# eriq-augustine/KB2E

Measured on AMD Instinct MI355X. Metric: training triples/sec (1/2/4/8 MI355X) + FB15k Hits@10(Filter), higher is better.
Workload: dtype f64

## Files before the change

### kb2e_amd/csrc/engine_transr_parallel.inc

```
namespace {

constexpr int32_t kRParLongMin = 128;

template <typename T, bool P, bool G>
const void* tile_fn(int nb) {
    switch (nb) {
        case 1: return (const void*)transr_tile_mfma_kernel<T, P, G, 1>;
        case 2: return (const void*)transr_tile_mfma_kernel<T, P, G, 2>;
        case 3: return (const void*)transr_tile_mfma_kernel<T, P, G, 3>;
        case 4: return (const void*)transr_tile_mfma_kernel<T, P, G, 4>;
        case 5: return (const void*)transr_tile_mfma_kernel<T, P, G, 5>;
        case 6: return (const void*)transr_tile_mfma_kernel<T, P, G, 6>;
        case 7: return (const void*)transr_tile_mfma_kernel<T, P, G, 7>;
        case 8: return (const void*)transr_tile_mfma_kernel<T, P, G, 8>;
    }
    throw std::runtime_error("TransR tile kernel: n > 128");
}

template <typename T>
const void* cons_tile_fn(int nb) {
    switch (nb) {
        case 1: return (const void*)transr_cons_tile_kernel<T, 1>;
        case 2: return (const void*)transr_cons_tile_kernel<T, 2>;
        case 3: return (const void*)transr_cons_tile_kernel<T, 3>;
// ... 214 lines not shown
        const std::pair<DevBuf*, DevBuf*> sets[] = {
            {&c->sb_x, &c->xreal}, {&c->sb_d, &c->aux}, {&c->sb_y, &c->rpar_y}, {&c->sb_wpart, &c->rpar_wpart},
            {&c->sb_rpart, &c->rpar_rpart}, {&c->sb_pflag, &c->rpar_pflag}, {&c->sb_cons_tile, &c->rpar_cons_tile},
            {&c->sb_cpairs, &c->rpar_cpairs}, {&c->sb_vio, &c->rpar_vio}, {&c->sb_cnrows, &c->rpar_cnrows}};
        for (const auto& pr : sets) {
            pr.first->free();
            if (c->sub > 1 && !c->rpar_merge_a && pr.second->p) {
                pr.first->alloc(pr.second->bytes);
                memset_sync(pr.first->p, 0, pr.first->bytes);
            }
        }
    }
    for (const void* k : {(const void*)rpar_scan_energy_kernel<double>, (const void*)rpar_scan_energy_kernel<float>,
                          (const void*)rpar_scan_energy_merged_kernel<double>,
                          (const void*)rpar_scan_energy_merged_kernel<float>})
        (void)hipFuncSetAttribute(k, hipFuncAttributeMaxDynamicSharedMemorySize, (int)rpar_scan_lds(c));
    (void)hipGetLastError();
}

void build_transr_tiles(kb2e_ctx* c, bool tiles, hipStream_t st, int set) {
    const int64_t nkeys = c->S * c->slots;
    rtile_count_kernel<<<1024, 256, 0, st>>>(c->keys_sorted.as<uint64_t>(), c->seg_start.as<int32_t>(),
                                                    c->nseg.as<int32_t>(), nkeys + 1, c->kl, c->cfg.num_entities,
                                                    c->rpar_St, c->rpar_ntiles.as<int32_t>(),
                                                    c->rpar_rel_begin.as<int32_t>());
    HIPCHK(hipGetLastError());
    if (!tiles) return;
    size_t tb = c->sort_tmp_bytes;
    HIPCHK(hipcub::DeviceScan::ExclusiveSum(c->sort_tmp.p, tb, c->rpar_ntiles.as<int32_t>(),
                                            c->rpar_tile_first.as<int32_t>(), (int)(nkeys + 1), st));
    rtile_scatter_kernel<<<1024, 256, 0, st>>>(c->rpar_ntiles.as<int32_t>(), c->rpar_tile_first.as<int32_t>(),
                                                      c->nseg.as<int32_t>(), c->rpar_tiles.as<RTile>());
    HIPCHK(hipGetLastError());
    if (c->rpar_brel.p) {
        rel_list_kernel<<<(int)c->nbi, 1024, 0, st>>>(c->rpar_rel_begin.as<int32_t>(), c->batch_seg.as<int32_t>(),
                                                     c->seg_row.as<int32_t>(), c->cfg.num_entities,
                                                     c->rel_order.as<int32_t>(), c->cfg.num_relations,
                                                     c->rpar_brel_cap, c->rpar_brel.as<int32_t>(),
                                                     c->rpar_bnrel.as<int32_t>());
        HIPCHK(hipGetLastError());
        HIPCHK(hipMemcpyAsync(c->pin_bnrel, c->rpar_bnrel.p, (size_t)c->nbi * 4, hipMemcpyDeviceToHost, st));
    }
    if (c->rpar_td_r.p) {
        RTileDescArgs d{};
        d.keys = c->keys_sorted.as<uint64_t>();
        d.seg_start = c->seg_start.as<int32_t>();
        d.seg_row = c->seg_row.as<int32_t>();
        d.tiles = c->rpar_tiles.as<RTile>();
        d.tile_first = c->rpar_tile_first.as<int32_t>();
        d.nseg = c->nseg.as<int32_t>();
        d.batch_seg = c->batch_seg.as<int32_t>();
        d.nb = (int32_t)c->nbi;
        d.sub = c->sub;
        d.Bs = (int32_t)c->Bs;
        d.St = c->rpar_St;
        d.ne = c->cfg.num_entities;
        d.B = (int32_t)c->B;
        d.kl = c->kl;
        d.si = c->si_[set].as<int32_t>();
        d.sj = c->sj_[set].as<int32_t>();
        d.side = c->side_[set].as<uint8_t>();
        d.heads = c->heads.as<int32_t>();
        d.tails = c->tails.as<int32_t>();
        d.batch_t0 = c->rpar_batch_t0.as<int32_t>();
        d.td_r = c->rpar_td_r.as<int32_t>();
        d.td_cnt = c->rpar_td_cnt.as<int32_t>();
        d.td_kk = c->rpar_td_kk.as<int32_t>();
        d.td_ent = c->rpar_td_ent.as<int32_t>();
        rtile_desc_kernel<<<2048, 256, 0, st>>>(d);
        HIPCHK(hipGetLastError());
    }
}

DevBuf& buf_set(int set, DevBuf& s0, DevBuf& s1) { return set ? s1 : s0; }

bool sub_overlap_on() {
    const char* e = getenv("KB2E_SUB_OVERLAP");
    return !(e && e[0] == '0');
}

int32_t pipe_opt_bits() {
    const char* e = getenv("KB2E_RPAR_PIPE_OPT");
    return e && e[0] ? (int32_t)(atoi(e) & kPipeOptAll) : kPipeOptAll;
}

constexpr int32_t kRecDeferChunks = 12;
int32_t rec_defer_chunks() {
    const char* e = getenv("KB2E_RPAR_REC_DEFER");
    return e && e[0] ? std::max(0, atoi(e)) : kRecDeferChunks;
}

template <typename T>
void fill_rpar(kb2e_ctx* c, int64_t b, int j, int set, RParArgs& a, RParBufs<T>& bf) {
    const int64_t ib = b * c->sub + j;
    const int64_t first = b * c->B + (int64_t)j * c->Bs;
    const int64_t cnt = std::min<int64_t>(c->Bs, c->B - (int64_t)j * c->Bs);
    a = RParArgs{};
    a.heads = c->heads.as<int32_t>();
    a.tails = c->tails.as<int32_t>();
    a.rels = c->rels.as<int32_t>();
    a.si = c->si() + first;
    a.sj = c->sj() + first;
    a.side = c->side() + first;
    a.B = (int32_t)cnt;
    a.n = c->n;
    a.ld = c->ld;
    a.ne = c->cfg.num_entities;
    a.nr = c->cfg.num_relations;
    a.St = c->rpar_St;
    a.tgroup = c->rpar_tgroup;
    a.batch = (int32_t)ib;
    a.lr = c->cfg.learning_rate;
    a.margin = c->cfg.margin;
    a.compat = c->cfg.transr_compat;
    a.l1 = c->cfg.distance == 0;
    a.keys = c->keys_sorted.as<uint64_t>();
    a.seg_start = c->seg_start.as<int32_t>();
    a.batch_seg = c->batch_seg.as<int32_t>();
    a.seg_row = c->seg_row.as<int32_t>();
    a.rel_begin = c->rpar_rel_begin.as<int32_t>();
    a.tile_first = c->rpar_tile_first.as<int32_t>();
    a.tiles = c->rpar_tiles.as<RTile>();
    a.kl = c->kl;
    a.act = c->act.as<uint8_t>() + first;
    a.loss = c->loss.as<double>() + first;
    a.proj = c->aux2.as<double>();
    a.tile_act = c->rpar_tile_act.as<int32_t>();
    a.batch_t0 = c->rpar_batch_t0.as<int32_t>();
    a.td_r = c->rpar_td_r.as<int32_t>();
    a.td_cnt = c->rpar_td_cnt.as<int32_t>();
    a.td_kk = c->rpar_td_kk.as<int32_t>();
    a.td_ent = c->rpar_td_ent.as<int32_t>();
    a.brel = c->rpar_brel.as<int32_t>() + ib * c->rpar_brel_cap;
    a.nrel = c->pin_bnrel[ib];
    if (a.nrel < 1 || a.nrel > c->rpar_brel_cap) throw std::logic_error("batch relation count out of range");
    bf = RParBufs<T>{};
    bf.ent = c->ent.as<T>();
    bf.rel = c->rel.as<T>();
    bf.W = c->w.as<T>();
    bf.x = buf_set(set, c->xreal, c->sb_x).as<T>();
    bf.d = buf_set(set, c->aux, c->sb_d).as<T>();
    bf.y = buf_set(set, c->rpar_y, c->sb_y).as<T>();
    bf.wpart = buf_set(set, c->rpar_wpart, c->sb_wpart).as<T>();
    bf.rpart = buf_set(set, c->rpar_rpart, c->sb_rpart).as<T>();
    bf.pair = c->rpar_pair.as<T>();
    bf.relpair = c->rpar_relpair.as<T>();
    bf.relpair_stamp = c->rpar_relpair_stamp.as<uint32_t>();
    bf.err = c->dataflow_err.as<uint32_t>() + 1;
    if (c->rpar_mfma) {
        bf.pflag = buf_set(set, c->rpar_pflag, c->sb_pflag).as<uint8_t>();
        bf.cons_tile = buf_set(set, c->rpar_cons_tile, c->sb_cons_tile).as<int32_t>();
        bf.cons_ppt = c->rpar_cons_wave ? kConsPpt : 1;
        bf.cpairs = buf_set(set, c->rpar_cpairs, c->sb_cpairs).as<int32_t>();
        bf.vio = buf_set(set, c->rpar_vio, c->sb_vio).as<int32_t>();
        bf.cnrows = buf_set(set, c->rpar_cnrows, c->sb_cnrows).as<int32_t>();
        bf.stats = getenv("KB2E_RPAR_STATS") != nullptr;
        bf.last_renorm = c->rpar_cons_seq ? 1 : 0;
        if (const char* dbg = getenv("KB2E_CONS_DBG")) bf.dbg = atoi(dbg);
        if (const char* cl = getenv("KB2E_RPAR_CHAIN_LIST")) bf.chain_list = std::max(64, atoi(cl));
        if (const char* ct = getenv("KB2E_RPAR_CHAIN_TILES")) bf.chain_tiles = std::max(1, atoi(ct));
        if (const char* rc = getenv("KB2E_RPAR_REC_CAP")) bf.rec_cap = std::max(4, atoi(rc));
        bf.pipe_opt = pipe_opt_bits();
        if (c->rpar_cons_seq) {
            bf.rec_stamp = bf.relpair_stamp + c->cfg.num_relations;
            bf.rec_defer = rec_defer_chunks();
        }
    }
    if (c->rpar_cons_wide || c->rpar_cons_gen || c->rpar_widep) {
        bf.pflag = buf_set(set, c->rpar_pflag, c->sb_pflag).as<uint8_t>();
        if (const char* dbg = getenv("KB2E_CONS_DBG")) bf.dbg = atoi(dbg);
        bf.stats = getenv("KB2E_RPAR_STATS") != nullptr;
        bf.last_renorm = 1;
    }
}

template <typename T>
void transr_phase_b(kb2e_ctx* c, RParArgs a, RParBufs<T> bf);

template <typename T>
void run_subbatch_transr_parallel(kb2e_ctx* c, int64_t b, int j) {
    const bool ov = c->sub > 1 && sub_overlap_on();
    const bool side = ov && j > 0;
    const int set = ov ? (j & 1) : 0;
    hipStream_t sa = side ? c->suba_stream : c->stream;
    RParArgs a;
    RParBufs<T> bf;
    fill_rpar<T>(c, b, j, set, a, bf);
    {
        unsigned long long* t0 = c->rpar_ptab.as<unsigned long long>();
        const size_t sz = (size_t)c->rpar_ptab_mask + 1;
        a.ptab = t0 + (c->batch_stamp % 3) * sz;
        a.ptab_next = t0 + ((c->batch_stamp + 1) % 3) * sz;
        a.ptab_mask = c->rpar_ptab_mask;
    }
    bf.stamp = ++c->batch_stamp;
    RParBufs<T> bfa = bf;
    if (c->sub > 1) {
        bfa.ent = c->snap_ent.as<T>();
        bfa.rel = c->snap_rel.as<T>();
        bfa.W = c->snap_w.as<T>();
    }
    if (side && j == 1) HIPCHK(hipStreamWaitEvent(sa, c->ev_adone[0], 0));
    if (side && j >= 2) HIPCHK(hipStreamWaitEvent(sa, c->ev_bdone[set], 0));
    auto a_done = [&] {
        if (!ov) return;
        HIPCHK(hipEventRecord(c->ev_adone[set], sa));
        if (side) HIPCHK(hipStreamWaitEvent(c->stream, c->ev_adone[set], 0));
    };
    auto b_done = [&] {
        if (ov) HIPCHK(hipEventRecord(c->ev_bdone[set], c->stream));
    };
    if (c->rpar_widep) {
        c->timed_on(sa, "score", [&] {
            wide_phase_a<T>(a, bfa, c->rpar_wg, c->rpar_max_tiles, c->rpar_scan.as<double>(),
                            c->rpar_scan_pre.as<double>(), c->transr_work.as<double>(),
                            c->transr_work_alt.as<double>(), sa);
        });
        if (c->cfg.transr_compat) std::swap(c->transr_work.p, c->transr_work_alt.p);
        a_done();
        c->timed("apply", [&] {
            wide_phase_b<T>(a, bf, c->rpar_wg, c->rpar_wsc.as<double>(), !c->rpar_no_constraint,
                            (int)std::min<int64_t>(c->cfg.num_relations, c->Bs), c->stream);
        });
        b_done();
        if (c->pending.size() > 4096) c->flush_timers();
        return;
    }
    const size_t lds = rpar_lds<T>(c);
    const int tgrid = c->rpar_max_tiles;
    const bool mf = c->rpar_mfma;
    const size_t lt = mf ? rmfma_lds<T>(c, false) : lds;
// ... 183 lines not shown
```

### kb2e_amd/csrc/kernels_transr_parallel.hpp

```cpp
#pragma once

#include <type_traits>

#include "kernels_common.hpp"

namespace kb2e {

struct RTile {
    int32_t seg, q;
};

struct RParArgs {
    const int32_t* heads;
    const int32_t* tails;
    const int32_t* rels;
    const int32_t* si;
    const int32_t* sj;
    const uint8_t* side;
    int32_t B, n, ld, ne, nr, St;
    int32_t batch;
    int32_t tgroup;
    double lr, margin;
    int32_t compat, l1;
    const uint64_t* keys;
// ... 62 lines not shown
__device__ __forceinline__ unsigned long long ptab_key(int r, int e) {
    return ((unsigned long long)r << kPtabEntBits) | (unsigned long long)e;
}
__device__ __forceinline__ uint32_t ptab_hash(int r, int e) {
    return ((uint32_t)e * 2654435761u) ^ ((uint32_t)r * 0x9E3779B1u + 0x7F4A7C15u);
}

__device__ __forceinline__ void ptab_insert(const RParArgs& a, int r, int e, int slot) {
    const unsigned long long key = ptab_key(r, e);
    const unsigned long long word = (key << kPtabSlotBits) | (unsigned long long)slot;
    uint32_t h = ptab_hash(r, e) & a.ptab_mask;
    while (true) {
        const unsigned long long old = atomicCAS(a.ptab + h, kPtabEmpty, word);
        if (old == kPtabEmpty) return;
        if ((old >> kPtabSlotBits) == key) {
            atomicMin(a.ptab + h, word);
            return;
        }
        h = (h + 1) & a.ptab_mask;
    }
}

__device__ __forceinline__ int ptab_first(const RParArgs& a, int r, int e) {
    const unsigned long long key = ptab_key(r, e);
    uint32_t h = ptab_hash(r, e) & a.ptab_mask;
    while (true) {
        const unsigned long long w = a.ptab[h];
        if (w == kPtabEmpty) return -1;
        if ((w >> kPtabSlotBits) == key) return (int)(w & ((1ull << kPtabSlotBits) - 1));
        h = (h + 1) & a.ptab_mask;
    }
}

__device__ __forceinline__ void ptab_clear_next(const RParArgs& a, int64_t tid, int64_t nthreads) {
    for (int64_t q = tid; q <= (int64_t)a.ptab_mask; q += nthreads) a.ptab_next[q] = kPtabEmpty;
}

__device__ __forceinline__ bool transr_pair_dup(const RParArgs& a, int slot, int r, int e) {
    return ptab_first(a, r, e) < slot;
}
__device__ __forceinline__ bool transr_relpair_dup(const RParArgs& a, int r) {
    return ptab_first(a, r, r) >= 0;
}

static __attribute__((unused)) __global__ __launch_bounds__(256) void transr_pair_first_kernel(RParArgs a) {
    const int slot = blockIdx.x * blockDim.x + threadIdx.x;
    ptab_clear_next(a, slot, (int64_t)gridDim.x * blockDim.x);
    if (slot >= 4 * a.B) return;
    const int kk = slot >> 2, u = (slot >> 1) & 1, role = slot & 1;
    if (!a.act[kk]) return;
    const int i0 = a.si[kk], jj = a.sj[kk];
    const int h = a.heads[i0], tt = a.tails[i0];
    const int hh = u ? (a.side[kk] ? h : jj) : h;
    const int th = u ? (a.side[kk] ? jj : tt) : tt;
    ptab_insert(a, a.rels[i0], role ? th : hh, slot);
}

template <typename T>
struct RParBufs {
    T* ent;
    T* rel;
    T* W;
    T* x;
    T* d;
    T* y;
    T* wpart;
    T* rpart;
    T* pair;
    T* relpair;
    uint32_t* relpair_stamp;
    uint32_t stamp;
    uint8_t* pflag;
    int32_t* cons_tile;
    int32_t cons_ppt;
    int32_t* cpairs;
    int32_t* cnrows;
    int32_t stats;
    int32_t last_renorm;
    int32_t dbg;
    int32_t chain_list;
    int32_t chain_tiles;
    int32_t rec_cap;
    int32_t pipe_opt;
    int32_t* vio;
    uint32_t* err;
    uint32_t* rec_stamp;
    int32_t rec_defer;
};

constexpr int32_t kPipeOptHandover = 2, kPipeOptDefer = 8, kPipeOptPublish = 16;
constexpr int32_t kPipeOptAll = kPipeOptHandover | kPipeOptDefer | kPipeOptPublish;

__host__ __device__ constexpr int rm_up16_host_dev(int v) { return (v + 15) & ~15; }
constexpr int kCPairs = 64;

struct RParMerge {
    int32_t sub;
    int32_t Bs;
    int32_t Blast;
    int32_t tcap;
    int32_t nch;
    int32_t brel_cap;
};

template <typename P>
__host__ __device__ __forceinline__ void rpar_advance(P*& p, int64_t k) {
    if (p) p += k;
}

template <typename T>
__host__ __device__ __forceinline__ void rpar_sub_view(RParArgs& a, RParBufs<T>& bf, const RParMerge& m, int j) {
    const int64_t s0 = (int64_t)j * m.Bs, t0 = (int64_t)j * m.tcap;
    a.B = j == m.sub - 1 ? m.Blast : m.Bs;
    a.batch += j;
    rpar_advance(a.si, s0);
    rpar_advance(a.sj, s0);
    rpar_advance(a.side, s0);
    rpar_advance(a.act, s0);
    rpar_advance(a.loss, s0);
    rpar_advance(a.proj, s0 * 4 * a.ld);
    rpar_advance(a.brel, (int64_t)j * m.brel_cap);
    rpar_advance(a.ptab, (int64_t)j * ((int64_t)a.ptab_mask + 1));
    rpar_advance(bf.x, s0 * 2 * a.ld);
    rpar_advance(bf.d, s0 * 2 * a.ld);
    rpar_advance(bf.y, s0 * 2 * a.ld);
    rpar_advance(bf.pflag, s0 * 4);
    rpar_advance(bf.wpart, t0 * bf.cons_ppt * a.n * a.ld);
    rpar_advance(bf.rpart, t0 * a.ld);
    rpar_advance(bf.cons_tile, t0 * bf.cons_ppt);
    rpar_advance(bf.cpairs, t0 * 2 * kCPairs);
    rpar_advance(bf.vio, t0 * kCPairs);
    rpar_advance(bf.cnrows, t0);
}

__device__ __forceinline__ void ptab_clear_group(const RParArgs& a, int sub, int64_t tid, int64_t nthreads) {
    const int64_t words = (int64_t)sub * ((int64_t)a.ptab_mask + 1);
    for (int64_t q = tid; q < words; q += nthreads) a.ptab_next[q] = kPtabEmpty;
}

template <typename T>
__host__ __device__ constexpr int rpar_lds_w(int n, int ld) {
    return n * ld;
}

__device__ __forceinline__ void tile_range(const RParArgs& a, int t, int& r, int& e0, int& cnt) {
    const RTile tl = a.tiles[t];
    const int p0 = a.seg_start[tl.seg], p1 = a.seg_start[tl.seg + 1];
    r = a.seg_row[tl.seg] - a.ne;
    const int ns = (p1 - p0) / 2;
    const int f = tl.q * a.St;
    e0 = p0 + 2 * f;
    cnt = min(a.St, ns - f);
}

template <typename T>
__device__ __forceinline__ void stage_matrix(T* Wl, const T* Wg, int n, int ld) {
    for (int idx = threadIdx.x; idx < n * ld; idx += blockDim.x) Wl[idx] = Wg[idx];
}

template <typename T>
__device__ __forceinline__ void project4(const T* Wl, int ld, int n, const T* v4 , T (&p)[4][2]) {
    const int l = lane_id();
    const int i = 2 * l;
#pragma unroll
    for (int q = 0; q < 4; ++q) p[q][0] = p[q][1] = T(0);
    if (i >= n) return;
    for (int j = 0; j < n; ++j) {
        const T w0 = Wl[j * ld + i], w1 = Wl[j * ld + i + 1];
#pragma unroll
        for (int q = 0; q < 4; ++q) {
            const T vj = v4[q * ld + j];
            p[q][0] += w0 * vj;
            p[q][1] += w1 * vj;
        }
// ... 369 lines not shown
        } else if (!transr_relpair_dup(a, r)) {
            ent = r;
        }
        ent_of[pq] = ent;
    }
    stage_matrix(Wl, bf.W + (int64_t)r * n * ld, n, ld);
    __syncthreads();
    T* v4 = vec + w * 4 * ld;
    const int i = 2 * l;
    for (int pq = w; pq < npairs; pq += 4) {
        const int ent = ent_of[pq];
        bool live = ent >= 0;
        for (int k = 0; live && k < pq; ++k) live = ent_of[k] != ent;
        T a0[2] = {T(0), T(0)}, G[2] = {T(0), T(0)}, da[2] = {T(0), T(0)};
        if (live) {
            lane_pair_load(bf.ent + (int64_t)ent * ld, n, a0);
            const T s0 = wave_sum(a0[0] * a0[0] + a0[1] * a0[1]);
            lane_pair_store(v4, n, a0);
            wave_lds_sync();
            T p[2] = {T(0), T(0)};
            if (i < n)
                for (int j = 0; j < n; ++j) {
                    const T aj = v4[j];
                    p[0] += Wl[j * ld + i] * aj;
                    p[1] += Wl[j * ld + i + 1] * aj;
                }
            if (i + 1 >= n) p[1] = T(0);
            if (i >= n) p[0] = T(0);
            wave_lds_sync();
            for (int m = 0; m < kRParMaxIter; ++m) {
                const T xx = wave_sum(p[0] * p[0] + p[1] * p[1]);
                if (!(xx > T(1))) break;
                G[0] += T(2) * p[0];
                G[1] += T(2) * p[1];
                lane_pair_store(v4, n, p);
                wave_lds_sync();
                T v[2];
                matvec_rows(Wl, ld, n, v4, v);
                lane_pair_store(v4 + ld, n, v);
                wave_lds_sync();
                T q[2] = {T(0), T(0)};
                if (i < n)
                    for (int j = 0; j < n; ++j) {
                        const T vj = v4[ld + j];
                        q[0] += Wl[j * ld + i] * vj;
                        q[1] += Wl[j * ld + i + 1] * vj;
                    }
                wave_lds_sync();
                const T c = T(2) * T(a.lr) * s0;
#pragma unroll
                for (int k = 0; k < 2; ++k) p[k] = i + k < n ? p[k] - T(2) * T(a.lr) * q[k] - c * p[k] : T(0);
            }
            lane_pair_store(v4, n, G);
            wave_lds_sync();
            matvec_rows(Wl, ld, n, v4, da);
            da[0] *= T(-a.lr);
            da[1] *= T(-a.lr);
            wave_lds_sync();
        }
        if (pq < 4 * cnt) {
            const int q = pq >> 2, u = (pq >> 1) & 1, role = pq & 1;
            const int kk = a.kl.kk_of(a.keys[e0 + 2 * q]);
            if (a.act[kk]) lane_pair_store(bf.pair + (((int64_t)kk * 2 + u) * 2 + role) * ld, n, da);
        } else {
            lane_pair_store(bf.relpair + (int64_t)r * ld, n, da);
            if (l == 0) bf.relpair_stamp[r] = bf.stamp;
        }
        const T dv[2] = {T(-a.lr) * a0[0], T(-a.lr) * a0[1]};
        lane_pair_store(Xl + pq * ld, n, G);
        lane_pair_store(Dl + pq * ld, n, dv);
    }
    __syncthreads();
    T* wp = bf.wpart + (int64_t)blockIdx.x * n * ld;
    for (int j = w; j < n; j += 4) {
        T acc[2];
        rank_sum_rows(Dl, Xl, npairs, ld, n, j, acc);
        lane_pair_store(wp + (int64_t)j * ld, n, acc);
    }
}

constexpr int kRParWaves = 16;

constexpr int kRecSteps = 4;
template <typename T>
__device__ __forceinline__ void rpar_record_convert(const RParArgs& a, const RParBufs<T>& bf, int r, T (&v)[2]) {
    typedef T T2 __attribute__((ext_vector_type(2)));
    const int n = a.n, l = lane_id();
    const T2* wrow = (const T2*)(bf.W + ((int64_t)r * n + (l < n ? l : 0)) * a.ld);
    const int nq = (n + 1) >> 1;
    T acc[4] = {T(0), T(0), T(0), T(0)};
    for (int q0 = 0; 2 * q0 < n; q0 += 2 * kRecSteps) {
        T2 x[2 * kRecSteps];
#pragma unroll
        for (int q = 0; q < 2 * kRecSteps; ++q) x[q] = wrow[q0 + q < nq ? q0 + q : nq - 1];
#pragma unroll
        for (int q = 0; q < 2 * kRecSteps; ++q) {
            const int i = 2 * (q0 + q);
            const T g0 = readlane_f(v[0], (q0 + q) & (kWave - 1)), g1 = readlane_f(v[1], (q0 + q) & (kWave - 1));
            acc[(2 * q) & 3] = fma(i < n ? x[q].x : T(0), g0, acc[(2 * q) & 3]);
            acc[(2 * q + 1) & 3] = fma(i + 1 < n ? x[q].y : T(0), g1, acc[(2 * q + 1) & 3]);
        }
    }
    const T da = -(T)a.lr * ((acc[0] + acc[1]) + (acc[2] + acc[3]));
    const T d0 = __shfl(da, (2 * l) & (kWave - 1)), d1 = __shfl(da, (2 * l + 1) & (kWave - 1));
    v[0] = 2 * l < n ? d0 : T(0);
    v[1] = 2 * l + 1 < n ? d1 : T(0);
}

__device__ __forceinline__ int rpar_entity_last(const RParArgs& a, int p0, int p1, int first, int stride) {
    const int l = lane_id();
    int last = -1;
    for (int base = p0 + first * kWave; base < p1; base += stride * kWave) {
        const int p = base + l;
        if (p < p1) {
            const uint64_t key = a.keys[p];
            const int kk = a.kl.kk_of(key);
            if (a.act[kk] && (key & (kRoleHead | kRoleTail))) last = max(last, kk * 2 + (int)((key >> 3) & 1));
        }
    }
#pragma unroll
    for (int s = 32; s >= 1; s >>= 1) last = max(last, __shfl_xor(last, s));
    return last;
}

template <typename T, bool GRAD>
__device__ __forceinline__ void rpar_entity_events(const RParArgs& a, const RParBufs<T>& bf, int row, int p0, int p1,
                                                   int first, int stride, int last, T (&acc)[2], T (&acc2)[2],
                                                   bool& dirty, bool& dirty2, bool& er_seen) {
    const int n = a.n, ld = a.ld, l = lane_id();
    const bool split = !GRAD && bf.last_renorm;
    const bool defer = !GRAD && bf.rec_stamp != nullptr;
    for (int base = p0 + first * kWave; base < p1; base += stride * kWave) {
        const int p = base + l;
        int src = -1;
        int src2 = -1;
        int rdef = -1;
        T c = T(0);
        bool nrm = false, er = false, post = false;
        if (p < p1) {
            const uint64_t key = a.keys[p];
            const int kk = a.kl.kk_of(key);
            if (a.act[kk]) {
                const int u = (int)((key >> 3) & 1);
                const uint32_t roles = (uint32_t)(key & 7);
                const bool hd = roles & kRoleHead, tl = roles & kRoleTail;
                er = roles & kRoleEntRel;
                if (GRAD) {
                    nrm = hd || tl;
                    if (hd != tl) {
                        src = kk * 2 + u;
                        c = (T)((hd ? -1.0 : 1.0) * (u ? 1.0 : -1.0) * a.lr);
                    }
                } else {
                    const int s0 = (kk * 2 + u) * 2;
                    const bool ph = hd && (!bf.pflag || bf.pflag[s0]);
                    const bool pt = tl && (!bf.pflag || bf.pflag[s0 + 1]);
                    nrm = ph || pt;
                    post = split && kk * 2 + u == last;
                    if (ph) src = s0;
                    if (pt) {
                        if (src < 0) src = s0 + 1;
                        else src2 = s0 + 1;
                    }
                    if (defer && src >= 0) {
                        const int r = a.rels[a.si[kk]];
                        if (bf.rec_stamp[r] == bf.stamp) rdef = r;
                    }
                }
            }
        }
        if (__ballot(nrm && !post)) dirty = true;
        if (__ballot(nrm && post)) dirty2 = true;
        if (__ballot(er)) er_seen = true;
        const T* tab = GRAD ? bf.y : bf.pair;
        for (int pass = 0; pass < (GRAD ? 1 : 2); ++pass) {
            const int mine = pass ? src2 : src;
            uint64_t m = __ballot(mine >= 0);
            const uint64_t pm = __ballot(post);
            while (m) {
                int ev[4];
                int k = 0;
                for (; k < 4 && m; ++k) {
                    ev[k] = __builtin_ctzll(m);
                    m &= m - 1;
                }
                T v[4][2];
#pragma unroll
                for (int q = 0; q < 4; ++q)
                    if (q < k) lane_pair_load(tab + (int64_t)readlane_i32(mine, ev[q]) * ld, n, v[q]);
                if (defer && __ballot(rdef >= 0)) {
#pragma unroll
                    for (int q = 0; q < 4; ++q)
                        if (q < k) {
                            const int rq = readlane_i32(rdef, ev[q]);
                            if (rq >= 0) rpar_record_convert<T>(a, bf, rq, v[q]);
                        }
                }
#pragma unroll
                for (int q = 0; q < 4; ++q)
                    if (q < k) {
                        const T cq = GRAD ? readlane_f(c, ev[q]) : T(1);
                        T(&dst)[2] = ((pm >> ev[q]) & 1) ? acc2 : acc;
                        dst[0] += cq * v[q][0];
                        dst[1] += cq * v[q][1];
                    }
            }
        }
    }
}

template <typename T, bool GRAD>
__device__ __forceinline__ void rpar_entity_finish(const RParArgs& a, const RParBufs<T>& bf, int row, T (&acc)[2],
                                                   T (&acc2)[2], bool dirty, bool dirty2, bool er_seen, int last) {
    const int n = a.n, ld = a.ld;
    const bool split = !GRAD && bf.last_renorm;
    if (!GRAD && er_seen && row < a.nr && bf.relpair_stamp[row] == bf.stamp) {
        T dv[2];
        lane_pair_load(bf.relpair + (int64_t)row * ld, n, dv);
        if (bf.rec_stamp && bf.rec_stamp[row] == bf.stamp) rpar_record_convert<T>(a, bf, row, dv);
        if (split && last < 0) {
            acc2[0] += dv[0];
            acc2[1] += dv[1];
            dirty2 = true;
        } else {
            acc[0] += dv[0];
            acc[1] += dv[1];
            dirty = true;
        }
    }
    if (!dirty && !dirty2) return;
    T* ptr = bf.ent + (int64_t)row * ld;
    T v[2];
    lane_pair_load(ptr, n, v);
    if (dirty) {
        v[0] += acc[0];
        v[1] += acc[1];
    }
    if (GRAD || (split && dirty)) {
        const T len = sqrt(wave_sum(v[0] * v[0] + v[1] * v[1]));
        v[0] = v[0] / len;
        v[1] = v[1] / len;
    }
    if (dirty2) {
        v[0] += acc2[0];
        v[1] += acc2[1];
    }
    lane_pair_store(ptr, n, v);
}

template <typename T, bool GRAD>
__device__ __forceinline__ void transr_entity_block(RParArgs a, RParBufs<T> bf, int32_t long_min, int bid, int G) {
    __shared__ T part[kRParWaves][4][kWave];
    __shared__ int flags[4];
    __shared__ int longs[1024], nlong;
    const int w = threadIdx.x >> 6, l = lane_id();
    const bool split = !GRAD && bf.last_renorm;
    const int s0 = a.batch_seg[a.batch], s1 = a.rel_begin[a.batch];
    const int blockIdx_x = bid;
    for (int c0 = s0 + blockIdx_x; c0 < s1; c0 += G * (int)blockDim.x) {
        if (threadIdx.x == 0) nlong = 0;
        __syncthreads();
        const int cs = c0 + G * (int)threadIdx.x;
        if (cs < s1 && a.seg_start[cs + 1] - a.seg_start[cs] >= long_min) longs[atomicAdd(&nlong, 1)] = cs;
        __syncthreads();
        const int nl = nlong;
        for (int li = 0; li < nl; ++li) {
        const int s = longs[li];
        const int p0 = a.seg_start[s], p1 = a.seg_start[s + 1];
        const int row = a.seg_row[s];
        if (threadIdx.x < 4) flags[threadIdx.x] = threadIdx.x == 3 ? -1 : 0;
        __syncthreads();
        int last = -1;
        if (split) {
            last = rpar_entity_last(a, p0, p1, w, kRParWaves);
            if (l == 0) atomicMax(&flags[3], last);
            __syncthreads();
            last = flags[3];
        }
        T acc[2] = {T(0), T(0)}, acc2[2] = {T(0), T(0)};
        bool dirty = false, dirty2 = false, er = false;
        rpar_entity_events<T, GRAD>(a, bf, row, p0, p1, w, kRParWaves, last, acc, acc2, dirty, dirty2,
                                    er);
        part[w][0][l] = acc[0];
        part[w][1][l] = acc[1];
        part[w][2][l] = acc2[0];
        part[w][3][l] = acc2[1];
        if (l == 0 && dirty) atomicOr(&flags[0], 1);
        if (l == 0 && er) atomicOr(&flags[1], 1);
        if (l == 0 && dirty2) atomicOr(&flags[2], 1);
        __syncthreads();
        if (w == 0) {
            acc[0] = part[0][0][l];
            acc[1] = part[0][1][l];
            acc2[0] = part[0][2][l];
            acc2[1] = part[0][3][l];
            for (int v = 1; v < kRParWaves; ++v) {
                acc[0] += part[v][0][l];
                acc[1] += part[v][1][l];
                acc2[0] += part[v][2][l];
                acc2[1] += part[v][3][l];
            }
            rpar_entity_finish<T, GRAD>(a, bf, row, acc, acc2, flags[0] != 0, flags[2] != 0, flags[1] != 0, last);
        }
        __syncthreads();
        }
    }
    for (int s = s0 + blockIdx_x * kRParWaves + w; s < s1; s += G * kRParWaves) {
        const int p0 = a.seg_start[s], p1 = a.seg_start[s + 1];
        if (p1 - p0 >= long_min) continue;
        const int row = a.seg_row[s];
        const int last = split ? rpar_entity_last(a, p0, p1, 0, 1) : -1;
        T acc[2] = {T(0), T(0)}, acc2[2] = {T(0), T(0)};
        bool dirty = false, dirty2 = false, er = false;
        rpar_entity_events<T, GRAD>(a, bf, row, p0, p1, 0, 1, last, acc, acc2, dirty, dirty2, er);
        rpar_entity_finish<T, GRAD>(a, bf, row, acc, acc2, dirty, dirty2, er, last);
    }
}

template <typename T, bool GRAD>
__global__ __launch_bounds__(1024) void transr_entity_kernel(RParArgs a, RParBufs<T> bf, int32_t long_min) {
    transr_entity_block<T, GRAD>(a, bf, long_min, blockIdx.x, gridDim.x);
}

template <typename T, bool PASS1, int RM>
__global__ __launch_bounds__(1024) void transr_rows_kernel(RParArgs a, RParBufs<T> bf, int32_t long_min,
                                                           int32_t egrid) {
    const int gw = (((int)blockIdx.x - egrid) * (int)blockDim.x + (int)threadIdx.x) >> 6;
    if ((int)blockIdx.x < egrid) transr_entity_block<T, PASS1>(a, bf, long_min, blockIdx.x, egrid);
    else if (RM == 4) transr_rel_rows4_wave<T, PASS1, 4>(a, bf, gw);
    else if (RM == 8) transr_rel_rows4_wave<T, PASS1, 8>(a, bf, gw);
    else transr_rel_rows_wave<T, PASS1>(a, bf, gw);
}

constexpr int kScanChunk = 64;

__device__ __forceinline__ void rpar_scan_sums_block(const double* proj, int64_t calls, int32_t ld, int32_t n,
                                                     double* sums, int c) {
    const int64_t c0 = (int64_t)c * kScanChunk, c1 = min<int64_t>(calls, c0 + kScanChunk);
    for (int e = threadIdx.x; e < 2 * n; e += blockDim.x) {
        const int side = e / n, i = e % n;
        double s[4] = {0, 0, 0, 0};
        for (int64_t k = c0; k < c1; k += 16) {
            double v[16];
#pragma unroll
            for (int q = 0; q < 16; ++q) v[q] = k + q < c1 ? proj[((k + q) * 2 + side) * ld + i] : 0.0;
#pragma unroll
            for (int q = 0; q < 16; ++q) s[q & 3] += v[q];
        }
        sums[(int64_t)c * 2 * n + e] = (s[0] + s[1]) + (s[2] + s[3]);
    }
}

static __attribute__((unused)) __global__ __launch_bounds__(256) void rpar_scan_sums_kernel(const double* proj, int64_t calls, int32_t ld,
                                                             int32_t n, double* sums) {
    rpar_scan_sums_block(proj, calls, ld, n, sums, blockIdx.x);
}

static __attribute__((unused)) __global__ __launch_bounds__(256) void rpar_scan_sums_merged_kernel(const double* proj, RParMerge m, int32_t ld,
                                                                    int32_t n, double* sums) {
    const int j = blockIdx.x / m.nch, c = blockIdx.x - j * m.nch;
    const int64_t calls = 2 * (int64_t)(j == m.sub - 1 ? m.Blast : m.Bs);
    rpar_scan_sums_block(proj + (int64_t)j * m.Bs * 4 * ld, calls, ld, n, sums + (int64_t)j * m.nch * 2 * n, c);
}

constexpr int kScanDirectMax = 256;

static __attribute__((unused)) __global__ __launch_bounds__(1024) void rpar_scan_prefix_kernel(
    const double* sums, int32_t nchunks, int32_t E2, const double* work_in, double* pre) {
    __shared__ double tot[32][33];
    const int el = threadIdx.x & 31, part = threadIdx.x >> 5;
    const int e = blockIdx.x * 32 + el;
    const int per = (nchunks + 31) / 32;
    const int c0 = part * per, c1 = min(nchunks, c0 + per);
    double s = 0.0;
    if (e < E2) {
        for (int c = c0; c < c1; c += 8) {
            double v[8];
#pragma unroll
            for (int q = 0; q < 8; ++q) v[q] = c + q < c1 ? sums[(int64_t)(c + q) * E2 + e] : 0.0;
#pragma unroll
            for (int q = 0; q < 8; ++q) s += v[q];
        }
    }
// ... 259 lines not shown
```

### kb2e_amd/csrc/kernels_transr_wave.hpp

```cpp
#pragma once

#include "kernels_transr_cons.hpp"

namespace kb2e {

template <int Q>
__device__ __forceinline__ float quad_bcast(float x) {
    return __int_as_float(__builtin_amdgcn_mov_dpp(__float_as_int(x), Q * 0x55, 0xF, 0xF, false));
}
template <int Q>
__device__ __forceinline__ double quad_bcast(double x) {
    const long long b = __double_as_longlong(x);
    const int lo = __builtin_amdgcn_mov_dpp((int)(b & 0xffffffff), Q * 0x55, 0xF, 0xF, false);
    const int hi = __builtin_amdgcn_mov_dpp((int)(b >> 32), Q * 0x55, 0xF, 0xF, false);
    return __longlong_as_double(((long long)hi << 32) | (unsigned)lo);
}

constexpr int kProjWaves = 2;

template <typename T>
__host__ __device__ constexpr int proj_wave_rows(int KS) {
    return sizeof(T) == 8 ? 4 * KS : 16 * ((KS + 3) / 4);
}

// ... 57 lines not shown
#pragma unroll
        for (int k = 0; k < 4; ++k) pf[4 * ib + k] = acc[k];
    }
    const bool upd = has && (which & 1);
    const int u = which >> 1;
    T xf[NS];
    T en = T(0);
    T* xrow = bf.x + ((int64_t)kk * 2 + u) * ld;
    T* drow = bf.d + ((int64_t)kk * 2 + u) * ld;
    double* prow = a.proj + ((int64_t)kk * 4 + which) * ld;
#pragma unroll
    for (int s = 0; s < NS; ++s) xf[s] = T(0);
#pragma unroll
    for (int s = 0; s < KS; ++s) {
        const int k = kmap<T>(s, kq);
        const T ph = (which & 2) ? quad_bcast<2>(pf[s]) : quad_bcast<0>(pf[s]);
        const T vh = (which & 2) ? quad_bcast<2>(vf[s]) : quad_bcast<0>(vf[s]);
        const T dp = pf[s] - ph - rf[s];
        en += a.l1 ? fabs(dp) : dp * dp;
        xf[s] = upd && k < n ? (a.l1 ? (dp > T(0) ? T(1) : T(-1)) : T(2) * dp) : T(0);
        if (upd && k < n) {
            xrow[k] = xf[s];
            drow[k] = vh - vf[s];
        }
        if (a.compat && has && k < n) prow[k] = (double)pf[s];
    }
    if (!a.compat) {
        const T er = row4_sum(en);
        const T ep = quad_bcast<1>(er);
        if (has && which == 3 && kq == 0) {
            const bool active = (double)ep + a.margin > (double)er;
            a.act[kk] = active ? 1 : 0;
            a.loss[kk] = active ? a.margin + (double)ep - (double)er : 0.0;
        }
        const T en3 = quad_bcast<3>(er);
        if (has && kq == 0 && (double)ep + a.margin > (double)en3) ptab_insert(a, r, e, kk * 4 + which);
    }
    T* yrow = bf.y + ((int64_t)kk * 2 + u) * ld;
#pragma unroll
    for (int jb = 0; jb < NB; ++jb) {
        typename M::acc_t acc = {T(0), T(0), T(0), T(0)};
#pragma unroll
        for (int s = 0; s < KS; ++s) {
            const int jr = jb * 16 + l16;
            acc = M::mma(jr < R ? Wl[jr * L + kmap<T>(s, kq)] : T(0), xf[s], acc);
        }
#pragma unroll
        for (int k = 0; k < 4; ++k) {
            const int j = jb * 16 + M::row(l, k);
            if (upd && j < n) yrow[j] = acc[k];
        }
    }
}

template <typename T, int KS>
__global__ __launch_bounds__(128) void transr_proj_wave_kernel(RParArgs a, RParBufs<T> bf) {
    if (!a.compat) ptab_clear_next(a, (int64_t)blockIdx.x * blockDim.x + threadIdx.x, (int64_t)gridDim.x * blockDim.x);
    transr_proj_wave_block<T, KS>(a, bf, blockIdx.x);
}

template <typename T, int KS>
__global__ __launch_bounds__(128) void transr_proj_wave_merged_kernel(RParArgs a, RParBufs<T> bf, RParMerge m) {
    if (!a.compat)
        ptab_clear_group(a, m.sub, (int64_t)blockIdx.x * blockDim.x + threadIdx.x, (int64_t)gridDim.x * blockDim.x);
    const int j = blockIdx.x / m.tcap;
    rpar_sub_view(a, bf, m, j);
    transr_proj_wave_block<T, KS>(a, bf, blockIdx.x - j * m.tcap);
}

template <typename T, int KS>
__device__ __forceinline__ void transr_grad_wave_block(const RParArgs& a, const RParBufs<T>& bf, int bid) {
    using M = Mfma16<T>;
    constexpr int NB = (KS + 3) / 4;
    constexpr int kOut = (NB * NB + kConsWaves - 1) / kConsWaves;
    constexpr int kSteps = 4;
    const int t = a.batch_t0[a.batch] + bid;
    if (t >= a.batch_t0[a.batch + 1]) return;
    const int r = a.td_r[t], cnt = a.td_cnt[t] & 255, single = (a.td_cnt[t] >> 8) & 1;
    const int n = a.n, ld = a.ld;
    const int w = threadIdx.x >> 6, l = lane_id(), kq = l >> 4, l16 = l & 15;
    const int nu = 2 * cnt;
    int rowu[kSteps];
    T cu[kSteps];
#pragma unroll
    for (int s = 0; s < kSteps; ++s) {
        const int u = 4 * s + kq;
        const int kk = a.td_kk[t * 8 + (u >> 1)], side = u & 1;
        rowu[s] = kk * 2 + side;
        cu[s] = (u < nu && a.act[kk]) ? (T)(-(side ? 1.0 : -1.0) * a.lr) : T(0);
    }
    T* const wp = bf.wpart + (int64_t)bid * n * ld;
#pragma unroll
    for (int q = 0; q < kOut; ++q) {
        const int tile = w + kConsWaves * q;
        if (tile >= NB * NB) break;
        const int jb = tile / NB, ib = tile % NB;
        const int j = jb * 16 + l16, i = ib * 16 + l16;
        T av[kSteps], bv[kSteps];
#pragma unroll
        for (int s = 0; s < kSteps; ++s) {
            av[s] = cu[s] * bf.d[(int64_t)rowu[s] * ld + (j < n ? j : 0)] * (j < n ? T(1) : T(0));
            bv[s] = bf.x[(int64_t)rowu[s] * ld + (i < n ? i : 0)] * (i < n ? T(1) : T(0));
        }
        typename M::acc_t acc = {T(0), T(0), T(0), T(0)};
#pragma unroll
        for (int s = 0; s < kSteps; ++s) acc = M::mma(av[s], bv[s], acc);
#pragma unroll
        for (int k = 0; k < 4; ++k) {
            const int jj = jb * 16 + M::row(l, k);
            if (jj < n && i < n) wp[(int64_t)jj * ld + i] = acc[k];
        }
        if (jb == 0) {
            typename M::acc_t dr = {T(0), T(0), T(0), T(0)};
#pragma unroll
            for (int s = 0; s < kSteps; ++s) dr = M::mma(l16 == 0 ? cu[s] : T(0), bv[s], dr);
            if (M::row(l, 0) == 0 && i < n) bf.rpart[(int64_t)bid * ld + i] = dr[0];
        }
    }
    if (w == 0) {
        const bool au = l < nu && a.act[a.td_kk[t * 8 + (l >> 1)]] != 0;
        const uint64_t m = __ballot(au);
        if (l == 0) a.tile_act[t] = __builtin_popcountll(m);
    }
    if (w == kConsWaves - 1) {
        __shared__ int ents[kCPairs];
        const RTile tl = a.tiles[t];
        bool relpair = false;
        if (tl.q == 0 && r < a.ne) {
            const int p0 = a.seg_start[tl.seg], ns = (a.seg_start[tl.seg + 1] - p0) / 2;
            for (int m0 = 0; m0 < ns && !relpair; m0 += kWave)
                relpair = __ballot(m0 + l < ns && a.act[a.kl.kk_of(a.keys[p0 + 2 * (m0 + l)])]) != 0;
        }
        const int pq = l;
        int ent = -1, slot = -1;
        if (pq < 4 * cnt) {
            const int q = pq >> 2, u = (pq >> 1) & 1, role = pq & 1;
            const int kk = a.td_kk[t * 8 + q];
            if (a.act[kk]) {
                slot = (kk * 2 + u) * 2 + role;
                const int e = a.td_ent[t * 32 + pq];
                if (!transr_pair_dup(a, slot, r, e)) ent = e;
            }
        } else if (pq == 4 * cnt && relpair && !transr_relpair_dup(a, r)) {
            ent = r;
            slot = -2;
        }
        ents[pq] = ent;
        wave_lds_sync();
        bool dup = false;
        for (int k = 0; k < kCPairs; k += 4) {
            const int4 e4 = *(const int4*)(ents + k);
            dup |= (k < pq && e4.x == ent) | (k + 1 < pq && e4.y == ent) | (k + 2 < pq && e4.z == ent) |
                   (k + 3 < pq && e4.w == ent);
        }
        const bool live = ent >= 0 && !dup;
        const uint64_t m = __ballot(live);
        const int pos = __builtin_popcountll(m & ((1ull << l) - 1));
        int32_t* cp = bf.cpairs + (int64_t)bid * 2 * kCPairs;
        if (live) {
            cp[pos] = ent;
            cp[kCPairs + pos] = slot;
        } else if (slot >= 0) {
            bf.pflag[slot] = 0;
        }
        if (l == 0) bf.cnrows[bid] = __builtin_popcountll(m) | (single << 7) | (r << 8);
    }
}

template <typename T, int KS>
__global__ __launch_bounds__(256) void transr_grad_wave_kernel(RParArgs a, RParBufs<T> bf) {
    transr_grad_wave_block<T, KS>(a, bf, blockIdx.x);
}

template <typename T, int KS>
__global__ __launch_bounds__(256) void transr_grad_wave_merged_kernel(RParArgs a, RParBufs<T> bf, RParMerge m) {
    const int j = blockIdx.x / m.tcap;
    rpar_sub_view(a, bf, m, j);
    transr_grad_wave_block<T, KS>(a, bf, blockIdx.x - j * m.tcap);
}

}
```

Before: 10.01 million.

## Deepen entity gather batching, skip inactive grad tiles, pair-vectorize wpart stores

In the GRAD entity-event loop, the batch of gathered rows per group grows from 4 to 16 so more loads are in flight at once. The GRAD cross-wave combine now reads five waves' partials before adding them, and it drops the unused acc2 sums. The TransR grad-wave kernel skips all tile work when no triple in the tile is active. It also swaps MFMA results between lanes with DPP so each lane writes two adjacent doubles as one vector store. The new paths are on by default behind an env bitmask. The cost is higher register pressure and some added lane-exchange overhead.

Result: faster. 10.16 million (median of 6 runs) (+1.5%).

```diff
diff --git a/kb2e_amd/csrc/engine_transr_parallel.inc b/kb2e_amd/csrc/engine_transr_parallel.inc
--- a/kb2e_amd/csrc/engine_transr_parallel.inc
+++ b/kb2e_amd/csrc/engine_transr_parallel.inc
@@ -320,6 +320,11 @@
 int32_t pipe_opt_bits() {
     const char* e = getenv("KB2E_RPAR_PIPE_OPT");
     return e && e[0] ? (int32_t)(atoi(e) & kPipeOptAll) : kPipeOptAll;
+}
+
+int32_t rows_opt_bits() {
+    const char* e = getenv("KB2E_RPAR_ROWS_OPT");
+    return e && e[0] ? (int32_t)(atoi(e) & kRowsOptAll) : kRowsOptAll;
 }
 
 constexpr int32_t kRecDeferChunks = 12;
@@ -385,6 +390,7 @@
     bf.relpair = c->rpar_relpair.as<T>();
     bf.relpair_stamp = c->rpar_relpair_stamp.as<uint32_t>();
     bf.err = c->dataflow_err.as<uint32_t>() + 1;
+    bf.rows_opt = rows_opt_bits();
     if (c->rpar_mfma) {
         bf.pflag = buf_set(set, c->rpar_pflag, c->sb_pflag).as<uint8_t>();
         bf.cons_tile = buf_set(set, c->rpar_cons_tile, c->sb_cons_tile).as<int32_t>();
diff --git a/kb2e_amd/csrc/kernels_transr_parallel.hpp b/kb2e_amd/csrc/kernels_transr_parallel.hpp
--- a/kb2e_amd/csrc/kernels_transr_parallel.hpp
+++ b/kb2e_amd/csrc/kernels_transr_parallel.hpp
@@ -168,6 +168,7 @@
     int32_t chain_tiles;
     int32_t rec_cap;
     int32_t pipe_opt;
+    int32_t rows_opt;
     int32_t* vio;
     uint32_t* err;
     uint32_t* rec_stamp;
@@ -176,6 +177,9 @@
 
 constexpr int32_t kPipeOptHandover = 2, kPipeOptDefer = 8, kPipeOptPublish = 16;
 constexpr int32_t kPipeOptAll = kPipeOptHandover | kPipeOptDefer | kPipeOptPublish;
+
+constexpr int32_t kRowsOptDeep = 2, kRowsOptStore = 4;
+constexpr int32_t kRowsOptAll = kRowsOptDeep | kRowsOptStore;
 
 __host__ __device__ constexpr int rm_up16_host_dev(int v) { return (v + 15) & ~15; }
 constexpr int kCPairs = 64;
@@ -711,6 +715,7 @@
 constexpr int kRParWaves = 16;
 
 constexpr int kRecSteps = 4;
+constexpr int kEntDeep = 16;
 template <typename T>
 __device__ __forceinline__ void rpar_record_convert(const RParArgs& a, const RParBufs<T>& bf, int r, T (&v)[2]) {
     typedef T T2 __attribute__((ext_vector_type(2)));
@@ -752,13 +757,49 @@
     return last;
 }
 
+template <typename T, bool GRAD, int D>
+__device__ __forceinline__ void rpar_entity_group(const RParArgs& a, const RParBufs<T>& bf, const T* tab, int mine, int rdef,
+                                                  T c, uint64_t& m, uint64_t pm, bool defer, T (&acc)[2], T (&acc2)[2]) {
+    const int n = a.n, ld = a.ld;
+    int ev[D];
+    int k = 0;
+#pragma unroll
+    for (int q = 0; q < D; ++q)
+        if (m) {
+            ev[q] = __builtin_ctzll(m);
+            m &= m - 1;
+            k = q + 1;
+        }
+    T v[D][2];
+#pragma unroll
+    for (int q = 0; q < D; ++q)
+        if (q < k) lane_pair_load(tab + (int64_t)readlane_i32(mine, ev[q]) * ld, n, v[q]);
+    if (defer && __ballot(rdef >= 0)) {
+#pragma unroll
+        for (int q = 0; q < D; ++q)
+            if (q < k) {
+                const int rq = readlane_i32(rdef, ev[q]);
+                if (rq >= 0) rpar_record_convert<T>(a, bf, rq, v[q]);
+            }
+    }
+#pragma unroll
+    for (int q = 0; q < D; ++q)
+        if (q < k) {
+            const T cq = GRAD ? readlane_f(c, ev[q]) : T(1);
+            T(&dst)[2] = ((pm >> ev[q]) & 1) ? acc2 : acc;
+            dst[0] += cq * v[q][0];
+            dst[1] += cq * v[q][1];
+        }
+}
+
 template <typename T, bool GRAD>
 __device__ __forceinline__ void rpar_entity_events(const RParArgs& a, const RParBufs<T>& bf, int row, int p0, int p1,
                                                    int first, int stride, int last, T (&acc)[2], T (&acc2)[2],
                                                    bool& dirty, bool& dirty2, bool& er_seen) {
-    const int n = a.n, ld = a.ld, l = lane_id();
+    const int l = lane_id();
     const bool split = !GRAD && bf.last_renorm;
     const bool defer = !GRAD && bf.rec_stamp != nullptr;
+    const bool deep = GRAD && (bf.rows_opt & kRowsOptDeep) != 0;
     for (int base = p0 + first * kWave; base < p1; base += stride * kWave) {
         const int p = base + l;
         int src = -1;
@@ -806,33 +847,10 @@
             const int mine = pass ? src2 : src;
             uint64_t m = __ballot(mine >= 0);
             const uint64_t pm = __ballot(post);
-            while (m) {
-                int ev[4];
-                int k = 0;
-                for (; k < 4 && m; ++k) {
-                    ev[k] = __builtin_ctzll(m);
-                    m &= m - 1;
-                }
-                T v[4][2];
-#pragma unroll
-                for (int q = 0; q < 4; ++q)
-                    if (q < k) lane_pair_load(tab + (int64_t)readlane_i32(mine, ev[q]) * ld, n, v[q]);
-                if (defer && __ballot(rdef >= 0)) {
-#pragma unroll
-                    for (int q = 0; q < 4; ++q)
-                        if (q < k) {
-                            const int rq = readlane_i32(rdef, ev[q]);
-                            if (rq >= 0) rpar_record_convert<T>(a, bf, rq, v[q]);
-                        }
-                }
-#pragma unroll
-                for (int q = 0; q < 4; ++q)
-                    if (q < k) {
-                        const T cq = GRAD ? readlane_f(c, ev[q]) : T(1);
-                        T(&dst)[2] = ((pm >> ev[q]) & 1) ? acc2 : acc;
-                        dst[0] += cq * v[q][0];
-                        dst[1] += cq * v[q][1];
-                    }
+            if (deep) {
+                while (m) rpar_entity_group<T, GRAD, kEntDeep>(a, bf, tab, mine, rdef, c, m, pm, defer, acc, acc2);
+            } else {
+                while (m) rpar_entity_group<T, GRAD, 4>(a, bf, tab, mine, rdef, c, m, pm, defer, acc, acc2);
             }
         }
     }
@@ -923,11 +941,29 @@
             acc[1] = part[0][1][l];
             acc2[0] = part[0][2][l];
             acc2[1] = part[0][3][l];
-            for (int v = 1; v < kRParWaves; ++v) {
-                acc[0] += part[v][0][l];
-                acc[1] += part[v][1][l];
-                acc2[0] += part[v][2][l];
-                acc2[1] += part[v][3][l];
+            if constexpr (GRAD) {
+                static_assert((kRParWaves - 1) % 5 == 0, "the combine reads five waves at a time");
+#pragma unroll 1
+                for (int v0 = 1; v0 < kRParWaves; v0 += 5) {
+                    T pv[5][2];
+#pragma unroll
+                    for (int v = 0; v < 5; ++v) {
+                        pv[v][0] = part[v0 + v][0][l];
+                        pv[v][1] = part[v0 + v][1][l];
+                    }
+#pragma unroll
+                    for (int v = 0; v < 5; ++v) {
+                        acc[0] += pv[v][0];
+                        acc[1] += pv[v][1];
+                    }
+                }
+            } else {
+                for (int v = 1; v < kRParWaves; ++v) {
+                    acc[0] += part[v][0][l];
+                    acc[1] += part[v][1][l];
+                    acc2[0] += part[v][2][l];
+                    acc2[1] += part[v][3][l];
+                }
             }
             rpar_entity_finish<T, GRAD>(a, bf, row, acc, acc2, flags[0] != 0, flags[2] != 0, flags[1] != 0, last);
         }
diff --git a/kb2e_amd/csrc/kernels_transr_wave.hpp b/kb2e_amd/csrc/kernels_transr_wave.hpp
--- a/kb2e_amd/csrc/kernels_transr_wave.hpp
+++ b/kb2e_amd/csrc/kernels_transr_wave.hpp
@@ -163,18 +163,23 @@
     const int nu = 2 * cnt;
     int rowu[kSteps];
     T cu[kSteps];
+    bool any_act = false;
 #pragma unroll
     for (int s = 0; s < kSteps; ++s) {
         const int u = 4 * s + kq;
         const int kk = a.td_kk[t * 8 + (u >> 1)], side = u & 1;
+        const bool au = u < nu && a.act[kk];
         rowu[s] = kk * 2 + side;
-        cu[s] = (u < nu && a.act[kk]) ? (T)(-(side ? 1.0 : -1.0) * a.lr) : T(0);
-    }
+        cu[s] = au ? (T)(-(side ? 1.0 : -1.0) * a.lr) : T(0);
+        any_act |= au;
+    }
+    const bool o_store = (bf.rows_opt & kRowsOptStore) != 0;
+    const bool skip = o_store && __ballot(any_act) == 0;
     T* const wp = bf.wpart + (int64_t)bid * n * ld;
 #pragma unroll
     for (int q = 0; q < kOut; ++q) {
         const int tile = w + kConsWaves * q;
-        if (tile >= NB * NB) break;
+        if (tile >= NB * NB || skip) break;
         const int jb = tile / NB, ib = tile % NB;
         const int j = jb * 16 + l16, i = ib * 16 + l16;
         T av[kSteps], bv[kSteps];
@@ -186,10 +191,27 @@
         typename M::acc_t acc = {T(0), T(0), T(0), T(0)};
 #pragma unroll
         for (int s = 0; s < kSteps; ++s) acc = M::mma(av[s], bv[s], acc);
-#pragma unroll
-        for (int k = 0; k < 4; ++k) {
-            const int jj = jb * 16 + M::row(l, k);
-            if (jj < n && i < n) wp[(int64_t)jj * ld + i] = acc[k];
+        if (o_store) {
+            typedef T T2 __attribute__((ext_vector_type(2)));
+            const bool odd = l & 1;
+            const T g0 = dpp_mov<0xB1>(odd ? acc[0] : acc[1]);
+            const T g1 = dpp_mov<0xB1>(odd ? acc[2] : acc[3]);
+            const int ic = i & ~1;
+#pragma unroll
+            for (int h = 0; h < 2; ++h) {
+                const int k = 2 * h + (odd ? 1 : 0);
+                const int jj = jb * 16 + M::row(l, k);
+                const T mine = acc[k], theirs = h ? g1 : g0;
+                T* const dst = wp + (int64_t)jj * ld + ic;
+                if (jj < n && ic + 1 < n) *(T2*)dst = odd ? T2{theirs, mine} : T2{mine, theirs};
+                else if (jj < n && ic < n) *dst = odd ? theirs : mine;
+            }
+        } else {
+#pragma unroll
+            for (int k = 0; k < 4; ++k) {
+                const int jj = jb * 16 + M::row(l, k);
+                if (jj < n && i < n) wp[(int64_t)jj * ld + i] = acc[k];
+            }
         }
         if (jb == 0) {
             typename M::acc_t dr = {T(0), T(0), T(0), T(0)};
```
